# jmaronas/TGP.pytorch

Measured on AMD Instinct MI355X. Metric: ELBO-steps/sec (N x M kernel + chol + flow), Power M=100 S=32, higher is better.
Workload: dtype f64; 1 GPU; tgp_power_tanh3x2; rows_per_gpu=8611, D=4, M=100, S=32, flow=tanh3x2, parallelism=row-shard x1, launch=hipgraph, 40 / 10 steps per graph launch, replicas=1

## Files before the change

tgp/pytorch_amd/csrc/tgp_dev.hpp:

```cpp
#pragma once
#include <utility>
#include <hip/hip_runtime.h>
#include <stdint.h>
#include "../../../include/tgp_hip.h"

typedef double d4 __attribute__((ext_vector_type(4)));
#define TGP_MFMA(a, b, c) __builtin_amdgcn_mfma_f64_16x16x4f64((a), (b), (c), 0, 0, 0)

#define TGP_ROWS_PER_BLOCK 64
#define TGP_TILE_LD 66
#define TGP_MAX_MT 8
#ifndef TGP_RSPLIT
#define TGP_RSPLIT 4
#endif
#define TGP_LOG_2PI_REF 1.8378770942368803

#ifdef TGP_STAMPS
#define TGP_STAMP(wsp, plan, i)                                                                       \
  do {                                                                                                \
    if (blockIdx.x == 0 && threadIdx.x == 0)                                                          \
      (wsp)[(plan).hdr + tgp::H_STAMP + (i)] = (double)__builtin_amdgcn_s_memrealtime();              \
  } while (0)
#else
#define TGP_STAMP(wsp, plan, i) \
// ... 21 lines not shown
  size_t nD;
  size_t Gp;
  size_t redp;
  size_t PP;
  int PPW;
  size_t dbg;
  size_t slabs;
  size_t total;
};

enum { H_S2 = 0, H_KL = 1, H_ETA = 2, H_EINV = 3, H_SIG_OS = 4, H_STEP = 5, H_STAMP = 8, H_PSTAMP = 32, H_OUT = 60, H_N = 64 };
enum { C_ELL = 0, C_ETAB = 1, C_SVB = 2, C_PAD = 3, C_THETA = 4 };

inline size_t rup(size_t x, size_t a) { return (x + a - 1) / a * a; }

inline int rows4_waves(int N, int MT) {
  if ((N + 15) / 16 + MT <= 255) return 4;
  if ((N + 31) / 32 + MT <= 255) return 8;
  return 0;
}
inline int rows_rw(int N) { return (N > 4000 && (N + 39) / 40 <= 256) ? 10 : 16; }
inline int plan_alloc_blocks(int N) {
  int nb = (N + TGP_ROWS_PER_BLOCK - 1) / TGP_ROWS_PER_BLOCK;
  const int nw = rows4_waves(N, 1);
  if (nw > 0 && (N + 4 * nw - 1) / (4 * nw) > nb) nb = (N + 4 * nw - 1) / (4 * nw);
  const int rw = rows_rw(N);
  if ((N + 4 * rw - 1) / (4 * rw) > nb) nb = (N + 4 * rw - 1) / (4 * rw);
  return nb < 1 ? 1 : nb;
}

inline int make_plan(Plan& p, int N, int D, int M, int S, int nblk, int P, int RP, int lik, int nw4 = 0, int rw = 16) {
  if (D < 1 || D > 16) return -2;
  if (M < 1 || M > 16 * TGP_MAX_MT) return TGP_E_UNSUPPORTED;
  p.N = N; p.D = D; p.M = M; p.S = S; p.nblk = nblk; p.P = P; p.RP = RP; p.lik = lik; p.nslots = 0; p.zs_lds = 0;
  p.MT = (M + 15) / 16; p.MP = p.MT * 16;
  p.DP = D <= 4 ? 4 : (D <= 8 ? 8 : 16);
  p.CT = (2 * p.DP + 1 + 15) / 16; p.CT16 = p.CT * 16;
  p.ntri = p.MT * (p.MT + 1) / 2;
  p.nw4 = nw4;
  p.rw = rw;
  p.rpb = nw4 > 0 ? 4 * nw4 : 4 * rw;
  p.nblocks = (N + p.rpb - 1) / p.rpb;
  if (p.nblocks < 1) p.nblocks = 1;
  p.slab_G = 0;
  p.slab_T = p.slab_G + (size_t)p.ntri * 256;
  p.slab_S = p.slab_T + (size_t)p.MP * p.CT16;
  p.slab_C = p.slab_S + p.MP;
  p.slab_len = rup(p.slab_C + C_THETA + P, 16);
  size_t o = 0;
  const size_t mm = (size_t)p.MP * p.MP;
  p.hdr = o; o += H_N;
  p.ils = o; o += 16;
  p.ls = o; o += 16;
  p.Zs = o; o += (size_t)p.MP * p.DP;
  p.mpad = o; o += p.MP;
  p.w = o; o += p.MP;
  p.tp = o; o += rup(P + 1, 16);
  p.tg = o; o += rup(P + 1, 16);
  p.Kmm = o; o += mm; p.L = o; o += mm; p.J = o; o += mm; p.LT = o; o += mm;
  p.Lq = o; o += mm; p.LqT = o; o += mm; p.S_ = o; o += mm; p.HpT = o; o += mm; p.Q = o; o += mm;
  p.nD = o; o += (size_t)p.MT * 256;
  p.Gp = o; o += mm;
  p.redp = o; o += p.slab_len;
  p.PPW = p.DP + 2;
  p.PP = o; o += (size_t)2 * p.MT * p.MP * p.PPW;
  p.dbg = o; o += 256;
  p.slabs = o; o += (size_t)p.nblocks * p.slab_len;
  p.total = o;
  return 0;
}


__device__ __forceinline__ double exp_fast(double x) {
  x = fmin(fmax(x, -745.0), 709.0);
  const double k = rint(x * 1.4426950408889634074);
  double r = fma(-k, 6.93147180369123816490e-01, x);
  r = fma(-k, 1.90821492927058770002e-10, r);
  const double r2 = r * r, r4 = r2 * r2, r8 = r4 * r4;
  const double p01 = 1.0 + r;
  const double p23 = fma(r, 1.0 / 6.0, 0.5);
  const double p45 = fma(r, 1.0 / 120.0, 1.0 / 24.0);
  const double p67 = fma(r, 1.0 / 5040.0, 1.0 / 720.0);
  const double p89 = fma(r, 1.0 / 362880.0, 1.0 / 40320.0);
  const double pab = fma(r, 1.0 / 39916800.0, 1.0 / 3628800.0);
  const double pcd = fma(r, 1.0 / 6227020800.0, 1.0 / 479001600.0);
  const double q0 = fma(p23, r2, p01), q1 = fma(p67, r2, p45), q2 = fma(pab, r2, p89);
  const double s0 = fma(q1, r4, q0), s1 = fma(pcd, r4, q2);
  return ldexp(fma(s1, r8, s0), (int)k);
}

#define TGP_SQRT3 1.7320508075688772
__device__ __forceinline__ double cov_value(int kernel, double s2, double d2) {
  if (kernel == TGP_KERNEL_SCALE_MATERN32) {
    const double ar = TGP_SQRT3 * sqrt(fmax(d2, 1e-30));
    return s2 * (1.0 + ar) * exp_fast(-ar);
  }
  return s2 * exp_fast(-0.5 * d2);
}
__device__ __forceinline__ double cov_gweight(int kernel, double s2, double d2) {
  if (kernel == TGP_KERNEL_SCALE_MATERN32) return 3.0 * s2 * exp_fast(-TGP_SQRT3 * sqrt(fmax(d2, 1e-30)));
  return s2 * exp_fast(-0.5 * d2);
}

__device__ __forceinline__ double rsqrt_nr_fwd(double d) {
  double y = __builtin_amdgcn_rsq(d);
  const double h = 0.5 * d;
  y = y * fma(-h * y, y, 1.5);
  y = y * fma(-h * y, y, 1.5);
  return y;
}

__device__ __forceinline__ double log_fast(double x) {
  double m = __builtin_amdgcn_frexp_mant(x);
  int e = __builtin_amdgcn_frexp_exp(x);
  const bool lo = m < 0.70710678118654752440;
  m = lo ? m + m : m;
  e = lo ? e - 1 : e;
  const double den = m + 1.0;
  double y = __builtin_amdgcn_rcp(den);
  y = fma(fma(-den, y, 1.0), y, y);
  y = fma(fma(-den, y, 1.0), y, y);
  const double num = m - 1.0;
  double s_ = num * y;
  s_ = fma(fma(-den, s_, num), y, s_);
  const double z = s_ * s_, z2 = z * z, z4 = z2 * z2;
  const double p01 = fma(z, 2.0 / 5.0, 2.0 / 3.0);
  const double p23 = fma(z, 2.0 / 9.0, 2.0 / 7.0);
  const double p45 = fma(z, 2.0 / 13.0, 2.0 / 11.0);
  const double p67 = fma(z, 2.0 / 17.0, 2.0 / 15.0);
  const double p8 = 2.0 / 19.0;
  const double q0 = fma(p23, z2, p01), q1 = fma(p67, z2, p45);
  const double P = fma(fma(p8, z4, q1), z4, q0);
  const double lm = fma(s_ * z, P, s_ + s_);
  const double ed = (double)e;
  return fma(ed, 6.93147180369123816490e-01, fma(ed, 1.90821492927058770002e-10, lm));
}

__device__ __forceinline__ double rcp_fast(double x) {
  double y = __builtin_amdgcn_rcp(x);
  y = fma(fma(-x, y, 1.0), y, y);
  y = fma(fma(-x, y, 1.0), y, y);
  return y;
}

__device__ __forceinline__ double softplus_d(double x) {
  if (x > 20.0) return x;
  const double e = exp_fast(x), u = 1.0 + e;
  if (u == 1.0) return e;
  return log_fast(u) * (e * rcp_fast(u - 1.0));
}
__device__ __forceinline__ double sigmoid_d(double x) { return 1.0 / (1.0 + exp_fast(-x)); }

#define TGP_EACH(u, N) _Pragma("unroll") for (int u = 0; u < (N); ++u)
template <int N>
__device__ __forceinline__ void exp_fast_n(double (&x)[N]) {
  double k[N], r[N], r2[N], r4[N], r8[N], p01[N], p23[N], p45[N], p67[N], p89[N], pab[N], pcd[N];
  TGP_EACH(u, N) x[u] = fmin(fmax(x[u], -745.0), 709.0);
  TGP_EACH(u, N) k[u] = rint(x[u] * 1.4426950408889634074);
  TGP_EACH(u, N) r[u] = fma(-k[u], 6.93147180369123816490e-01, x[u]);
  TGP_EACH(u, N) r[u] = fma(-k[u], 1.90821492927058770002e-10, r[u]);
  TGP_EACH(u, N) r2[u] = r[u] * r[u];
  TGP_EACH(u, N) p01[u] = 1.0 + r[u];
  TGP_EACH(u, N) p23[u] = fma(r[u], 1.0 / 6.0, 0.5);
  TGP_EACH(u, N) p45[u] = fma(r[u], 1.0 / 120.0, 1.0 / 24.0);
  TGP_EACH(u, N) p67[u] = fma(r[u], 1.0 / 5040.0, 1.0 / 720.0);
  TGP_EACH(u, N) p89[u] = fma(r[u], 1.0 / 362880.0, 1.0 / 40320.0);
  TGP_EACH(u, N) pab[u] = fma(r[u], 1.0 / 39916800.0, 1.0 / 3628800.0);
  TGP_EACH(u, N) pcd[u] = fma(r[u], 1.0 / 6227020800.0, 1.0 / 479001600.0);
  TGP_EACH(u, N) r4[u] = r2[u] * r2[u];
  TGP_EACH(u, N) p01[u] = fma(p23[u], r2[u], p01[u]);
  TGP_EACH(u, N) p45[u] = fma(p67[u], r2[u], p45[u]);
  TGP_EACH(u, N) p89[u] = fma(pab[u], r2[u], p89[u]);
  TGP_EACH(u, N) r8[u] = r4[u] * r4[u];
  TGP_EACH(u, N) p01[u] = fma(p45[u], r4[u], p01[u]);
  TGP_EACH(u, N) p89[u] = fma(pcd[u], r4[u], p89[u]);
  TGP_EACH(u, N) x[u] = ldexp(fma(p89[u], r8[u], p01[u]), (int)k[u]);
}
template <int N>
__device__ __forceinline__ void rcp_fast_n(double (&x)[N]) {
  double y[N];
  TGP_EACH(u, N) y[u] = __builtin_amdgcn_rcp(x[u]);
  TGP_EACH(u, N) y[u] = fma(fma(-x[u], y[u], 1.0), y[u], y[u]);
  TGP_EACH(u, N) x[u] = fma(fma(-x[u], y[u], 1.0), y[u], y[u]);
}
template <int N>
__device__ __forceinline__ void rsqrt_nr_fwd_n(const double (&d)[N], double (&y)[N]) {
  TGP_EACH(u, N) y[u] = __builtin_amdgcn_rsq(d[u]);
  TGP_EACH(u, N) y[u] = y[u] * fma(-(0.5 * d[u]) * y[u], y[u], 1.5);
  TGP_EACH(u, N) y[u] = y[u] * fma(-(0.5 * d[u]) * y[u], y[u], 1.5);
}
template <int N>
__device__ __forceinline__ void log_fast_n(double (&x)[N]) {
  double m[N], den[N], y[N], num[N], s_[N], z[N], z2[N], z4[N], p01[N], p23[N], p45[N], p67[N], ed[N];
  TGP_EACH(u, N) {
    m[u] = __builtin_amdgcn_frexp_mant(x[u]);
    int e = __builtin_amdgcn_frexp_exp(x[u]);
    const bool lo = m[u] < 0.70710678118654752440;
    m[u] = lo ? m[u] + m[u] : m[u];
    e = lo ? e - 1 : e;
    ed[u] = (double)e;
  }
  TGP_EACH(u, N) den[u] = m[u] + 1.0;
  TGP_EACH(u, N) num[u] = m[u] - 1.0;
  TGP_EACH(u, N) y[u] = __builtin_amdgcn_rcp(den[u]);
  TGP_EACH(u, N) y[u] = fma(fma(-den[u], y[u], 1.0), y[u], y[u]);
  TGP_EACH(u, N) y[u] = fma(fma(-den[u], y[u], 1.0), y[u], y[u]);
  TGP_EACH(u, N) s_[u] = num[u] * y[u];
  TGP_EACH(u, N) s_[u] = fma(fma(-den[u], s_[u], num[u]), y[u], s_[u]);
  TGP_EACH(u, N) z[u] = s_[u] * s_[u];
  TGP_EACH(u, N) z2[u] = z[u] * z[u];
  TGP_EACH(u, N) p01[u] = fma(z[u], 2.0 / 5.0, 2.0 / 3.0);
  TGP_EACH(u, N) p23[u] = fma(z[u], 2.0 / 9.0, 2.0 / 7.0);
  TGP_EACH(u, N) p45[u] = fma(z[u], 2.0 / 13.0, 2.0 / 11.0);
  TGP_EACH(u, N) p67[u] = fma(z[u], 2.0 / 17.0, 2.0 / 15.0);
  TGP_EACH(u, N) z4[u] = z2[u] * z2[u];
  TGP_EACH(u, N) p01[u] = fma(p23[u], z2[u], p01[u]);
  TGP_EACH(u, N) p45[u] = fma(p67[u], z2[u], p45[u]);
  TGP_EACH(u, N) p45[u] = fma(2.0 / 19.0, z4[u], p45[u]);
  TGP_EACH(u, N) p01[u] = fma(p45[u], z4[u], p01[u]);
  TGP_EACH(u, N) p01[u] = fma(s_[u] * z[u], p01[u], s_[u] + s_[u]);
  TGP_EACH(u, N) x[u] = fma(ed[u], 6.93147180369123816490e-01, fma(ed[u], 1.90821492927058770002e-10, p01[u]));
}

__device__ __forceinline__ double xor_sum16(double x) {
  const unsigned lo = __double2loint(x), hi = __double2hiint(x);
  const auto a = __builtin_amdgcn_permlane16_swap(lo, lo, false, false);
  const auto b = __builtin_amdgcn_permlane16_swap(hi, hi, false, false);
  return __hiloint2double(b[0], a[0]) + __hiloint2double(b[1], a[1]);
}
__device__ __forceinline__ double xor_sum32(double x) {
  const unsigned lo = __double2loint(x), hi = __double2hiint(x);
  const auto a = __builtin_amdgcn_permlane32_swap(lo, lo, false, false);
  const auto b = __builtin_amdgcn_permlane32_swap(hi, hi, false, false);
  return __hiloint2double(b[0], a[0]) + __hiloint2double(b[1], a[1]);
}
__device__ __forceinline__ double quad_sum(double x) { return xor_sum32(xor_sum16(x)); }
template <int R>
__device__ __forceinline__ double ror_sum(double x) {
  const int lo = __double2loint(x), hi = __double2hiint(x);
  const int l2 = __builtin_amdgcn_update_dpp(0, lo, 0x120 + R, 0xf, 0xf, false);
  const int h2 = __builtin_amdgcn_update_dpp(0, hi, 0x120 + R, 0xf, 0xf, false);
  return x + __hiloint2double(h2, l2);
}
__device__ __forceinline__ double wave_sum(double x) {
  x = xor_sum16(xor_sum32(x));
  return ror_sum<1>(ror_sum<2>(ror_sum<4>(ror_sum<8>(x))));
}

template <int K>
__device__ __forceinline__ double bcast_row_k(double x) {
  return __builtin_amdgcn_update_dpp(0.0, x, 0x150 + K, 0xf, 0xf, true);
}
template <class F, int... Is>
__device__ __forceinline__ void static_for_impl(F&& f, std::integer_sequence<int, Is...>) {
  (f(std::integral_constant<int, Is>{}), ...);
}
template <int N, class F>
__device__ __forceinline__ void static_for(F&& f) {
  static_for_impl(static_cast<F&&>(f), std::make_integer_sequence<int, N>{});
}

__device__ __forceinline__ double rsqrt_nr(double d) {
  double y = __builtin_amdgcn_rsq(d);
  const double h = 0.5 * d;
  y = y * fma(-h * y, y, 1.5);
  y = y * fma(-h * y, y, 1.5);
  return y;
}

__device__ __forceinline__ int potrf_trtri16(double (&a)[16], double (&x)[16], int lane) {
  int bad = 0;
  static_for<16>([&](auto kc) {
    constexpr int k = decltype(kc)::value;
    const double d = bcast_row_k<k>(a[k]);
    if (!(d > 0.0) && bad == 0) bad = k + 1;
    const double rinv = rsqrt_nr(d);
    double s0 = 0.0, s1 = 0.0;
    static_for<16>([&](auto mc) {
      constexpr int m = decltype(mc)::value;
      if constexpr (m < k) {
        if constexpr ((m & 1) == 0) s0 = fma(bcast_row_k<k>(a[m]), x[m], s0);
        else s1 = fma(bcast_row_k<k>(a[m]), x[m], s1);
      }
    });
    x[k] = (lane == k) ? rinv : (lane < k ? -(s0 + s1) * rinv : 0.0);
    a[k] = (lane == k) ? d * rinv : a[k] * rinv;
    static_for<16>([&](auto jc) {
      constexpr int j = decltype(jc)::value;
      if constexpr (j > k) {
        a[j] = fma(-a[k], bcast_row_k<j>(a[k]), a[j]);
        asm volatile("" : "+v"(a[j]));
      }
    });
  });
  return bad;
}

template <bool PANEL, bool TRTRI = false, bool RDIAG = false>
__device__ __forceinline__ int potrf_panel16(double (&dg)[16], double (&a)[16], double* x = nullptr, int lane = 0,
                                             double* rd = nullptr) {
  int bad = 0;
  static_for<16>([&](auto kc) {
    constexpr int k = decltype(kc)::value;
    const double d = bcast_row_k<k>(dg[k]);
    if (!(d > 0.0) && bad == 0) bad = k + 1;
    const double rinv = rsqrt_nr(d);
// ... 818 lines not shown
```

tgp/pytorch_amd/csrc/tgp_mm.hip:

```cpp
#include "tgp_dev.hpp"
#include "tgp_prep.hpp"
#include "tgp_launch.hpp"

namespace tgp {

#define PREP_THREADS 512
#ifndef TGP_W4_WINDOWS
#define TGP_W4_WINDOWS 2
#endif

__global__ __launch_bounds__(PREP_THREADS) void k_prep_a(Plan p, tgp_model md, FlowProg fp, double* __restrict__ ws,
                                                         int32_t* __restrict__ status) {
  extern __shared__ __attribute__((aligned(16))) unsigned char smem_raw[];
  double* sm = reinterpret_cast<double*>(smem_raw);
  const int tid = threadIdx.x, lane = tid & 63;
  const int wave = __builtin_amdgcn_readfirstlane(tid >> 6);
  const int r = lane & 15, q = lane >> 4;
  const int M = p.M, D = p.D, MP = p.MP, DP = p.DP, MT = p.MT;

  int32_t* sy = status + 4;
  const int nb_total = 3 + MT * MT;
  if ((int)blockIdx.x < MT * MT) {
    prep_tile_role<PREP_THREADS, true>(p, md, ws, (int)blockIdx.x, sy);
    sync_leave(sy, nb_total);
    return;
  }

  if ((int)blockIdx.x == MT * MT) {
    prep_xform_role<PREP_THREADS, false>(p, md, fp, ws);
    sync_leave(sy, nb_total);
    return;
  }

  const int cb = (int)blockIdx.x - (MT * MT + 1);
  constexpr int NW = PREP_THREADS / 64;
  const int LD = MP + 1;
  double* A = sm;
  double* zs = sm + (size_t)MP * LD;
  __shared__ int s_info, s_nan, s_next, s_sync;
  __shared__ double s_ils[16];
  if (tid == 0) { s_info = 0; s_nan = 0; s_next = 0; s_sync = 0; }
  int tbase = 0;
  if (tid < 16) s_ils[tid] = tid < D ? 1.0 / softplus_d(md.raw_ls[tid]) : 0.0;
  const double s2 = softplus_d(md.raw_os[0]);
  const bool zl = p.zs_lds != 0;
  if (zl) {
    for (int i = tid; i < MP * DP; i += PREP_THREADS) {
      const int mrow = i / DP, d = i % DP;
      zs[i] = (mrow < M && d < D) ? md.Z[(size_t)mrow * D + d] * (1.0 / softplus_d(md.raw_ls[d])) : 0.0;
    }
  }
  __syncthreads();
  bool has_nan = false;
  double jit = md.jitter;
  auto kmm_elem = [&](int rr, int cc) {
    double k;
    if (rr < M) {
      double d2 = 0.0;
      if (zl) {
        for (int d = 0; d < DP; d += 4) {
          const double2 a0 = *reinterpret_cast<const double2*>(zs + rr * DP + d), a1 = *reinterpret_cast<const double2*>(zs + rr * DP + d + 2);
          const double2 b0 = *reinterpret_cast<const double2*>(zs + cc * DP + d), b1 = *reinterpret_cast<const double2*>(zs + cc * DP + d + 2);
          const double t0 = a0.x - b0.x, t1 = a0.y - b0.y, t2 = a1.x - b1.x, t3 = a1.y - b1.y;
          d2 += t0 * t0; d2 += t1 * t1; d2 += t2 * t2; d2 += t3 * t3;
        }
      } else {
        for (int d = 0; d < D; ++d) {
          const double tt = (md.Z[(size_t)rr * D + d] - md.Z[(size_t)cc * D + d]) * s_ils[d];
          d2 += tt * tt;
        }
      }
      k = s2 * exp_fast(-0.5 * d2);
      has_nan |= (k != k);
      if (rr == cc) k += jit;
    } else {
      k = (rr == cc) ? 1.0 : 0.0;
    }
    return k;
  };
  auto ll_sum = [&](int i0, int j0, int kbeg, int kend) {
    d4 acc = {0, 0, 0, 0};
    return tile_mm_f([&](int k) { return A[(i0 + r) * LD + k + q]; }, [&](int k) { return A[(j0 + r) * LD + k + q]; }, kbeg,
                     kend, acc);
  };
  auto write_L = [&](int ti, int tj) {
#pragma unroll
    for (int u = 0; u < 4; ++u) {
      const int rr = 16 * ti + q + 4 * u, cc = 16 * tj + r;
      ws[p.L + (size_t)rr * MP + cc] = (ti != tj || cc <= rr) ? A[rr * LD + cc] : 0.0;
      const int rt = 16 * tj + q + 4 * u, ct = 16 * ti + r;
      ws[p.LT + (size_t)rt * MP + ct] = (ti != tj || rt <= ct) ? A[ct * LD + rt] : 0.0;
    }
  };
  auto inv_diag = [&](int jt) {
    const int li = lane & 15;
    double dgv[16], xv[16];
#pragma unroll
    for (int c = 0; c < 16; ++c) dgv[c] = A[(16 * jt + li) * LD + 16 * jt + c];
    trtri16(dgv, xv, li);
#pragma unroll
    for (int u = 0; u < 4; ++u) {
      const double xv4 = q == 0 ? xv[4 * u] : (q == 1 ? xv[4 * u + 1] : (q == 2 ? xv[4 * u + 2] : xv[4 * u + 3]));
      ws[p.nD + jt * 256 + (4 * u + q) * 16 + li] = -xv4;
    }
  };
  auto sub16 = [&](int i, int c, int k0) {
    double a4[4], b4[4];
#pragma unroll
    for (int s4 = 0; s4 < 4; ++s4) { a4[s4] = A[(16 * i + r) * LD + k0 + 4 * s4 + q]; b4[s4] = A[(16 * c + r) * LD + k0 + 4 * s4 + q]; }
    double cur[4];
#pragma unroll
    for (int rr = 0; rr < 4; ++rr) cur[rr] = A[(16 * i + q + 4 * rr) * LD + 16 * c + r];
    d4 acc = {0, 0, 0, 0};
#pragma unroll
    for (int s4 = 0; s4 < 4; ++s4) acc = TGP_MFMA(a4[s4], b4[s4], acc);
#pragma unroll
    for (int rr = 0; rr < 4; ++rr) A[(16 * i + q + 4 * rr) * LD + 16 * c + r] = cur[rr] - acc[rr];
  };
  const double* __restrict__ Kg = ws + p.Kmm;
  bool tiles_seen = false;
  auto fill_tile = [&](int i, int c, int ncol) {
    double kv[4];
    if (c >= 2) {
      if (!tiles_seen) {
        const int v = sync_wait(sy + SY_TILES, [&](int x) { return (x & 0xffff) >= MT * MT; });
        if (v == (int)0x80000000 && lane == 0) s_sync = 1;
        tiles_seen = true;
      }
#pragma unroll
      for (int u = 0; u < 4; ++u) kv[u] = ld_agent(Kg + (size_t)(16 * i + q + 4 * u) * MP + 16 * c + r);
#pragma unroll
      for (int u = 0; u < 4; ++u) {
        const int rr = 16 * i + q + 4 * u, cc = 16 * c + r;
        has_nan |= (kv[u] != kv[u]);
        if (rr == cc) kv[u] = rr < M ? kv[u] + jit : 1.0;
      }
    } else if (zl) {
      const int cc = 16 * c + r;
      double e[4];
      TGP_EACH(u, 4) {
        const int rr = 16 * i + q + 4 * u;
        double d2 = 0.0;
        for (int d = 0; d < DP; d += 4) {
          const double2 a0 = *reinterpret_cast<const double2*>(zs + rr * DP + d), a1 = *reinterpret_cast<const double2*>(zs + rr * DP + d + 2);
          const double2 b0 = *reinterpret_cast<const double2*>(zs + cc * DP + d), b1 = *reinterpret_cast<const double2*>(zs + cc * DP + d + 2);
          const double t0 = a0.x - b0.x, t1 = a0.y - b0.y, t2 = a1.x - b1.x, t3 = a1.y - b1.y;
          d2 += t0 * t0; d2 += t1 * t1; d2 += t2 * t2; d2 += t3 * t3;
        }
        e[u] = -0.5 * d2;
      }
      exp_fast_n<4>(e);
      TGP_EACH(u, 4) {
        const int rr = 16 * i + q + 4 * u;
        double k = s2 * e[u];
        has_nan |= (rr < M) && (k != k);
        if (rr == cc) k += jit;
        kv[u] = rr < M ? k : (rr == cc ? 1.0 : 0.0);
      }
    } else {
#pragma unroll
      for (int u = 0; u < 4; ++u) kv[u] = kmm_elem(16 * i + q + 4 * u, 16 * c + r);
    }
    if (ncol > 0) {
      const d4 upd = ll_sum(16 * i, 16 * c, 0, 16 * ncol);
#pragma unroll
      for (int u = 0; u < 4; ++u) kv[u] -= upd[u];
    }
#pragma unroll
    for (int u = 0; u < 4; ++u) A[(16 * i + q + 4 * u) * LD + 16 * c + r] = kv[u];
  };
#define PREP_BARRIER() asm volatile("s_waitcnt lgkmcnt(0)\n\ts_barrier" ::: "memory")
#ifdef TGP_STAMPS
  double tph[10] = {0, 0, 0, 0, 0, 0, 0, 0, 0, 0};
  double tcnt[6] = {0, 0, 0, 0, 0, 0};
  unsigned long long tl_ = 0;
#define PSTAMP0() do { __builtin_amdgcn_sched_barrier(0); tl_ = __builtin_amdgcn_s_memtime(); __builtin_amdgcn_sched_barrier(0); } while (0)
#define PSTAMP(i) do { __builtin_amdgcn_sched_barrier(0); unsigned long long tn_ = __builtin_amdgcn_s_memtime(); __builtin_amdgcn_sched_barrier(0); tph[i] += (double)(tn_ - tl_); tl_ = tn_; } while (0)
#else
#define PSTAMP0() do { } while (0)
#define PSTAMP(i) do { } while (0)
#endif
  int attempt = 0;
  PSTAMP0();
  for (;; ++attempt) {
    if (wave < MT) fill_tile(wave, 0, 0);
    PREP_BARRIER();
    PSTAMP(0);
    for (int j = 0; j < MT; ++j) {
      const int j0 = 16 * j;
      const int npan = (MT - 1 - j) * 16;
      const int npw = npan > 64 ? 2 : (npan > 0 ? 1 : 0);
      double ltile[4] = {0.0, 0.0, 0.0, 0.0};
      bool did_diag = false;
      if (wave < npw || (npw == 0 && wave == 0)) {
        __builtin_amdgcn_s_setprio(3);
        const int li = lane & 15, l0 = wave * 64 + lane;
        const bool has = l0 < npan;
        const int prow = j0 + (npan > 0 ? 16 : 0) + (has ? l0 : 0);
        double dg[16], a[16];
#pragma unroll
        for (int c = 0; c < 16; ++c) dg[c] = A[(j0 + li) * LD + j0 + c];
        if (npan > 0) {
#pragma unroll
          for (int c = 0; c < 16; ++c) a[c] = A[prow * LD + j0 + c];
        }
#ifdef TGP_STAMPS
        asm volatile("s_waitcnt lgkmcnt(0)" ::: "memory");
#endif
        PSTAMP(1);
        int bad = 0;
        if (npan > 0) bad = potrf_panel16<true>(dg, a);
        else bad = potrf_panel16<false>(dg, a);
#ifdef TGP_STAMPS
        asm volatile("" ::"v"(dg[15]), "v"(a[15]));
#endif
        PSTAMP(2);
        if (has && npan > 0) {
#pragma unroll
          for (int c = 0; c < 16; ++c) A[prow * LD + j0 + c] = a[c];
        }
        if (wave == 0) {
#pragma unroll
          for (int u = 0; u < 4; ++u)
            ltile[u] = q == 0 ? dg[4 * u] : (q == 1 ? dg[4 * u + 1] : (q == 2 ? dg[4 * u + 2] : dg[4 * u + 3]));
          did_diag = true;
          if (lane == 0 && bad != 0 && s_info == 0) s_info = j0 + bad;
        }
#ifdef TGP_STAMPS
        asm volatile("s_waitcnt lgkmcnt(0)" ::: "memory");
#endif
        PSTAMP(3);
        __builtin_amdgcn_s_setprio(0);
#ifdef TGP_STAMPS
        if (wave != 0) { tph[j == 0 ? 7 : 8] += tph[1] + tph[2] + tph[3]; tph[1] = tph[2] = tph[3] = 0.0; }
#endif
      } else if (wave != 4 || j < TGP_W4_WINDOWS) {
        const int nt = (j >= 1 && ((j - 1) & 1) == cb) ? 1 : 0;
        const int nf = MT - 1 - j;
        const int nwl = (j + 1 - cb) / 2;
        const int ntask = nt + nf + nwl;
        for (;;) {
          int t = 0;
          if (lane == 0) t = atomicAdd(&s_next, 1);
          t = __builtin_amdgcn_readfirstlane(t) - tbase;
          if (t >= ntask) break;
          if (t < nt) { inv_diag(j - 1); continue; }
          t -= nt;
          if (t < nf) { fill_tile(j + 1 + t, j + 1, j); continue; }
          t -= nf;
          write_L(j - 1, 2 * t + cb);
        }
#ifdef TGP_STAMPS
        asm volatile("s_waitcnt lgkmcnt(0)" ::: "memory");
        if (j == 0) PSTAMP(7); else PSTAMP(8);
#endif
      }
      tbase += ((j >= 1 && ((j - 1) & 1) == cb) ? 1 : 0) + (MT - 1 - j) + (j + 1 - cb) / 2 +
               (NW - (j < TGP_W4_WINDOWS ? 0 : 1) - (npw > 0 ? npw : 1));
      PREP_BARRIER();
      PSTAMP(4);
      if (did_diag) {
#pragma unroll
        for (int u = 0; u < 4; ++u) A[(j0 + (lane & 15)) * LD + j0 + 4 * u + q] = ltile[u];
      }
      if (j + 1 < MT) {
        for (int i = j + 1 + wave; i < MT; i += NW) sub16(i, j + 1, j0);
#ifdef TGP_STAMPS
        asm volatile("s_waitcnt lgkmcnt(0)" ::: "memory");
#endif
        PSTAMP(5);
        PREP_BARRIER();
        PSTAMP(6);
      }
    }
    if (has_nan) s_nan = 1;
    __syncthreads();
    if (s_info == 0 || s_nan != 0 || !(md.jitter_ladder > 0.0) || attempt == 3) break;
    __syncthreads();
    if (tid == 0) s_info = 0;
    jit = md.jitter + md.jitter_ladder * (attempt == 0 ? 1.0 : (attempt == 1 ? 10.0 : 100.0));
    __syncthreads();
  }
  if (((MT - 1) & 1) == cb && wave == NW - 1) inv_diag(MT - 1);
  for (int t = wave; t < (MT + 1 - cb) / 2; t += NW) write_L(MT - 1, 2 * t + cb);
  PSTAMP(9);
#ifdef TGP_STAMPS
  if (lane == 0) {
    if (wave == 0)
      for (int i = 0; i < 10; ++i) ws[p.hdr + H_PSTAMP + i] = tph[i];
    if (wave == 3) for (int i = 1; i <= 5; ++i) { ws[p.hdr + H_PSTAMP + 26 + i] = tph[i]; ws[p.hdr + 20 + i] = tcnt[i]; }
    ws[p.hdr + H_PSTAMP + 10 + 2 * wave] = tph[7];
    ws[p.hdr + H_PSTAMP + 11 + 2 * wave] = tph[8];
  }
#endif
  if (tid == 0 && cb == 0) {
    status[0] = s_sync != 0 ? TGP_STATUS_SYNC_TIMEOUT : s_info;
    if (s_sync != 0) __hip_atomic_fetch_add(status + 3, 1, __ATOMIC_RELAXED, __HIP_MEMORY_SCOPE_AGENT);
    status[1] = s_nan;
    status[2] = s_info == 0 ? attempt : 0;
  }
  sync_leave(sy, nb_total);
#undef PREP_BARRIER
}

size_t prep_a_lds_bytes(const Plan& p) {
  return ((size_t)p.MP * (p.MP + 1) + (p.zs_lds ? (size_t)p.MP * p.DP : 0) + 16) * sizeof(double);
}

#define RED_ELEMS (256 / TGP_RSPLIT)
__global__ __launch_bounds__(256) void k_reduce(Plan p, double* __restrict__ ws) {
#ifdef TGP_STAMPS
  if (blockIdx.x == 0 && threadIdx.x == 0) ws[p.dbg + 200 + 16] = (double)__builtin_amdgcn_s_memrealtime();
#endif
  __shared__ double part_s[TGP_RSPLIT][RED_ELEMS];
  const int tid = threadIdx.x, sh = tid / RED_ELEMS, el = tid % RED_ELEMS;
  const size_t e = (size_t)blockIdx.x * RED_ELEMS + el;
  const bool in = e < p.slab_len;
  const int b0 = (int)((long long)p.nblocks * sh / TGP_RSPLIT), b1 = (int)((long long)p.nblocks * (sh + 1) / TGP_RSPLIT);
  const double* sl = ws + p.slabs + (in ? e : 0);
  constexpr int RB = 28;
  double s0 = 0.0, s1 = 0.0, s2 = 0.0, s3 = 0.0;
  for (int b = b0; b < b1; b += RB) {
    double t[RB];
#pragma unroll
    for (int u = 0; u < RB; ++u) {
      const int bu = b + u < b1 ? b + u : b1 - 1;
      t[u] = sl[(size_t)bu * p.slab_len];
    }
#pragma unroll
    for (int u = 0; u < RB; ++u) t[u] = b + u < b1 ? t[u] : 0.0;
#pragma unroll
    for (int u = 0; u < RB; u += 4) { s0 += t[u]; s1 += t[u + 1]; s2 += t[u + 2]; s3 += t[u + 3]; }
  }
  part_s[sh][el] = b1 > b0 ? (s0 + s1) + (s2 + s3) : 0.0;
  __syncthreads();
  if (sh != 0 || !in) return;
  double s = 0.0;
#pragma unroll
  for (int k = 0; k < TGP_RSPLIT; ++k) s += part_s[k][el];
  if (e < p.slab_T) {
    const int t = (int)(e >> 8), in_t = (int)(e & 255), row = in_t >> 4, col = in_t & 15;
    int ti = 0;
    while ((ti + 1) * (ti + 2) / 2 <= t) ++ti;
    const int tj = t - ti * (ti + 1) / 2;
    if (ti == tj && col > row) return;
    double* G = ws + p.Gp;
    st_wt(&G[(size_t)(ti * 16 + row) * p.MP + tj * 16 + col], s);
    st_wt(&G[(size_t)(tj * 16 + col) * p.MP + ti * 16 + row], s);
  } else {
    st_wt(&ws[p.redp + e], s);
  }
}

__device__ __forceinline__ double red_tail(const Plan& p, const double* __restrict__ ws, size_t e) { return ws[p.redp + e]; }

#define BWD_THREADS 512
#define TGP_PF2 32

__device__ __forceinline__ void adam_elem(const AdamDev& A, long i, double g, double pi, double mi, double vi, double bc1,
                                          double bc2s) {
  const double gi = A.sign * g;
  const double m1 = A.b1 * mi + (1.0 - A.b1) * gi;
  const double v1 = A.b2 * vi + (1.0 - A.b2) * gi * gi;
  A.m[i] = m1;
  A.v[i] = v1;
  A.p[i] = pi - (A.lr / bc1) * m1 / (sqrt(v1) / bc2s + A.eps);
}

enum { SB_PROG = 0, SB_LEFT = 1 };
#ifdef TGP_STAMPS
#define BW_STAMP(on, i) do { if ((on) && threadIdx.x == 0) ws[p.dbg + 200 + (i)] = (double)__builtin_amdgcn_s_memrealtime(); } while (0)
#else
#define BW_STAMP(on, i) do { } while (0)
#endif

__device__ __forceinline__ void bwd_leave(int32_t* sb) {
  __syncthreads();
  if (threadIdx.x == 0) sync_add(sb + SB_LEFT, 1);
}

__device__ __forceinline__ void report_sync_timeout(int32_t* __restrict__ status) {
  __hip_atomic_store(status, (int32_t)TGP_STATUS_SYNC_TIMEOUT, __ATOMIC_RELAXED, __HIP_MEMORY_SCOPE_AGENT);
  __hip_atomic_fetch_add(status + 3, 1, __ATOMIC_RELAXED, __HIP_MEMORY_SCOPE_AGENT);
}
template <class P>
__device__ __forceinline__ void bwd_wait(const int32_t* w, P pred, int32_t* __restrict__ status) {
  if (threadIdx.x < 64) {
    const int v = sync_wait(w, pred);
    if (v == (int)0x80000000 && threadIdx.x == 0) {
      report_sync_timeout(status);
      asm volatile("s_waitcnt vmcnt(0)" ::: "memory");
    }
  }
  __syncthreads();
}
__device__ __forceinline__ bool bwd_timed_out(const int32_t* __restrict__ status) {
  return __hip_atomic_load(status, __ATOMIC_RELAXED, __HIP_MEMORY_SCOPE_AGENT) == (int32_t)TGP_STATUS_SYNC_TIMEOUT;
}

typedef double bwd_d2 __attribute__((ext_vector_type(2)));
#define BWD_G_NIT ((8 * TGP_MAX_MT * 16 + BWD_THREADS - 1) / BWD_THREADS)
__device__ __forceinline__ void bwd_g_issue(const Plan& p, const double* __restrict__ ws, int c0,
                                            bwd_d2 (&gv)[BWD_G_NIT], double& sv0) {
  const int MP = p.MP, tid = threadIdx.x;
  const double* __restrict__ Gp = ws + p.Gp;
#pragma unroll
  for (int u = 0; u < BWD_G_NIT; ++u) {
    const int i = tid + u * BWD_THREADS;
    const int ic = i < MP * 8 ? i : 0;
    gv[u] = *reinterpret_cast<const bwd_d2*>(Gp + (size_t)(ic >> 3) * MP + c0 + 2 * (ic & 7));
  }
  sv0 = tid < 16 ? red_tail(p, ws, p.slab_S + c0 + tid) : 0.0;
}
__device__ __forceinline__ void bwd_g_commit(const Plan& p, double* Gs, double* LbL, double* svL,
                                             const bwd_d2 (&gv)[BWD_G_NIT], double sv0) {
  const int MP = p.MP, tid = threadIdx.x;
#pragma unroll
  for (int u = 0; u < BWD_G_NIT; ++u) {
    const int i = tid + u * BWD_THREADS;
    if (i < MP * 8) {
      reinterpret_cast<bwd_d2*>(Gs)[i] = gv[u];
      reinterpret_cast<bwd_d2*>(LbL)[i] = bwd_d2{0.0, 0.0};
    }
  }
  if (tid < 16) svL[tid] = sv0;
}

template <int PF, bool SWAP = false, class FB>
__device__ __forceinline__ d4 tile_mm_regA(const double (&a)[PF], FB fb, int n, d4 acc) {
#pragma unroll
  for (int s0 = 0; s0 < PF; s0 += 8) {
    if (s0 < n) {
      double o[8];
#pragma unroll
      for (int u = 0; u < 8; ++u) o[u] = s0 + u < n ? fb(s0 + u) : 0.0;
#pragma unroll
      for (int u = 0; u < 8; ++u)
        if (s0 + u < n) acc = SWAP ? TGP_MFMA(o[u], a[s0 + u], acc) : TGP_MFMA(a[s0 + u], o[u], acc);
    }
  }
  return acc;
}

__device__ __forceinline__ void bwd_lam_role(const Plan& p, const tgp_model& md, const tgp_grads& g, double* __restrict__ ws,
                                             const AdamDev& ad, double* sm, int c, const int32_t* __restrict__ status) {
  static_assert(TGP_MAX_MT <= BWD_THREADS / 64, "one tile per wave");
  const int MP = p.MP, MT = p.MT, M = p.M;
  double* Gs = sm;
  double* LbL = Gs + (size_t)MP * 16;
  double* svL = LbL + (size_t)MP * 16;
  const int tid = threadIdx.x, lane = tid & 63, wave = __builtin_amdgcn_readfirstlane(tid >> 6), r = lane & 15, q = lane >> 4;
  const int c0 = 16 * c;
  BW_STAMP(c == 0, 4);
  bwd_d2 gv[BWD_G_NIT];
  double sv0;
  bwd_g_issue(p, ws, c0, gv, sv0);
  constexpr int PF = TGP_PF2;
  const double* __restrict__ Lq = ws + p.Lq;
  const int j = wave, j0 = 16 * j;
// ... 422 lines not shown
  __syncthreads();
  for (int i = tid; i < N2 * D; i += 256) {
    const int c = i / D, d = i - c * D;
    zT[d * N2 + c] = X2[i] * ils[d];
  }
  for (int i = tid; i < nr * D; i += 256) {
    const int r = i / D, d = i - r * D;
    xT[d * COVF_ROWS + r] = X1[n0 * D + i] * ils[d];
  }
  __syncthreads();
  const double s2 = ils[16];
  const int npairs = nr * (N2 / 2);
  const int sr = 512 / N2, sc = 512 - sr * N2;
  int e = 2 * tid, r = e / N2, c = e - r * N2;
  double* __restrict__ Ko = K + n0 * (long)N2;
  for (int p = tid; p < npairs; p += 512) {
    int r1 = r + sr, c1 = c + sc;
    if (c1 >= N2) { c1 -= N2; ++r1; }
    const bool has1 = p + 256 < npairs;
    const int rb = has1 ? r1 : r, cb = has1 ? c1 : c;
    double ev[4] = {0.0, 0.0, 0.0, 0.0};
    for (int d = 0; d < D; ++d) {
      const double xa = xT[d * COVF_ROWS + r], xb = xT[d * COVF_ROWS + rb];
      const double2 za = *reinterpret_cast<const double2*>(zT + d * N2 + c);
      const double2 zb = *reinterpret_cast<const double2*>(zT + d * N2 + cb);
      const double t0 = xa - za.x, t1 = xa - za.y, t2 = xb - zb.x, t3 = xb - zb.y;
      ev[0] += t0 * t0; ev[1] += t1 * t1; ev[2] += t2 * t2; ev[3] += t3 * t3;
    }
    if (kernel == TGP_KERNEL_SCALE_RBF) {
      TGP_EACH(u, 4) ev[u] *= -0.5;
      exp_fast_n<4>(ev);
      TGP_EACH(u, 4) ev[u] *= s2;
    } else {
      TGP_EACH(u, 4) ev[u] = cov_value(kernel, s2, ev[u]);
    }
    if (self) {
      if (n0 + r == c) ev[0] += jitter;
      if (n0 + r == c + 1) ev[1] += jitter;
      if (n0 + rb == cb) ev[2] += jitter;
      if (n0 + rb == cb + 1) ev[3] += jitter;
    }
    *reinterpret_cast<double2*>(Ko + e) = make_double2(ev[0], ev[1]);
    if (has1) *reinterpret_cast<double2*>(Ko + e + 512) = make_double2(ev[2], ev[3]);
    r = r1 + sr; c = c1 + sc;
    if (c >= N2) { c -= N2; ++r; }
    e += 1024;
  }
}

__global__ __launch_bounds__(256) void k_kl(const double* __restrict__ m, const double* __restrict__ Lam, int M,
                                             double* __restrict__ out, double* __restrict__ g_m,
                                             double* __restrict__ g_Lam) {
  __shared__ double wsum[4];
  const int tid = threadIdx.x;
  double part = 0.0;
  for (int it = tid; it < M * M; it += 256) {
    const int r = it / M, c = it % M;
    double gl = 0.0;
    if (c <= r) {
      const double x = Lam[it];
      part += x * x;
      gl = x;
      if (c == r) { part -= log(x * x); gl = x - 1.0 / x; }
    }
    if (g_Lam) g_Lam[it] = gl;
  }
  for (int i = tid; i < M; i += 256) {
    part += m[i] * m[i];
    if (g_m) g_m[i] = m[i];
  }
  part = wave_sum(part);
  if ((tid & 63) == 0) wsum[tid >> 6] = part;
  __syncthreads();
  if (tid == 0) out[0] = 0.5 * (wsum[0] + wsum[1] + wsum[2] + wsum[3] - (double)M);
}

__global__ void k_unpad(const double* __restrict__ src, int MP, int M, double* __restrict__ dst) {
  const int i = blockIdx.x * blockDim.x + threadIdx.x;
  if (i >= M * M) return;
  dst[i] = src[(size_t)(i / M) * MP + i % M];
}

__global__ __launch_bounds__(PREP_THREADS) void k_chol_only(const double* __restrict__ Ain, int M, int MP,
                                                            double* __restrict__ Lout, double* __restrict__ Jout,
                                                            int32_t* __restrict__ status) {
  extern __shared__ __attribute__((aligned(16))) unsigned char smem_raw[];
  double* A = reinterpret_cast<double*>(smem_raw);
  const int LD = MP + 1;
  double* dinv = A + (size_t)MP * LD;
  __shared__ int s_info, s_nan;
  const int tid = threadIdx.x;
  if (tid == 0) { s_info = 0; s_nan = 0; }
  __syncthreads();
  bool has_nan = false;
  for (int i = tid; i < M * M; i += PREP_THREADS) {
    const double x = Ain[i];
    has_nan |= (x != x);
    A[(i / M) * LD + i % M] = x;
  }
  if (has_nan) s_nan = 1;
  for (int j = 0; j < M; ++j) {
    __syncthreads();
    const double d = A[j * LD + j];
    if (!(d > 0.0)) {
      if (tid == 0 && s_info == 0) s_info = j + 1;
    }
    const double dj = sqrt(d), inv = 1.0 / dj;
    __syncthreads();
    for (int i = j + tid; i < M; i += PREP_THREADS) A[i * LD + j] = (i == j) ? dj : A[i * LD + j] * inv;
    __syncthreads();
    const int rem = M - j - 1;
    for (int e = tid; e < rem * rem; e += PREP_THREADS) {
      const int i = j + 1 + e / rem, k = j + 1 + e % rem;
      if (k <= i) A[i * LD + k] -= A[i * LD + j] * A[k * LD + j];
    }
  }
  __syncthreads();
  if (tid < M) dinv[tid] = 1.0 / A[tid * LD + tid];
  __syncthreads();
  if (Jout != nullptr && tid < M) {
    const int c = tid;
    for (int i = c + 1; i < M; ++i) {
      double s = A[i * LD + c] * dinv[c];
      for (int k = c + 1; k < i; ++k) s += A[i * LD + k] * A[c * LD + k];
      A[c * LD + i] = -s * dinv[i];
    }
  }
  __syncthreads();
  for (int i = tid; i < M * M; i += PREP_THREADS) {
    const int r = i / M, c = i % M;
    double l = 0.0, jv = 0.0;
    if (c < r) { l = A[r * LD + c]; jv = A[c * LD + r]; }
    else if (c == r) { l = A[r * LD + r]; jv = dinv[r]; }
    Lout[i] = l;
    if (Jout != nullptr) Jout[i] = jv;
  }
  if (tid == 0) { status[0] = s_info; status[1] = s_nan; }
}

#define LAUNCH_CHECK()                                   \
  do {                                                   \
    hipError_t e_ = hipGetLastError();                   \
    if (e_ != hipSuccess) return set_error(e_, __FILE__, __LINE__); \
  } while (0)

int launch_prepare(const Plan& p_in, const tgp_model& md, const FlowProg& fp, double* ws, int32_t* status,
                   hipStream_t st) {
  Plan p = p_in;
  p.zs_lds = 1;
  if (prep_a_lds_bytes(p) > 160 * 1024 - 1024) p.zs_lds = 0;
  const size_t lds = prep_a_lds_bytes(p);
  static size_t lds_cur = 48 * 1024;
  if (int rc = ensure_lds(reinterpret_cast<const void*>(k_prep_a), lds, &lds_cur)) return rc;
  hipLaunchKernelGGL(k_prep_a, dim3(3 + p.MT * p.MT), dim3(PREP_THREADS), lds, st, p, md, fp, ws, status);
  LAUNCH_CHECK();
  return 0;
}

int launch_backward_mm(const Plan& p, const tgp_model& md, const tgp_grads& g, double* out, double* ws, int32_t* status,
                       hipStream_t st, const AdamDev* adam) {
  const AdamDev ad = adam != nullptr ? *adam : AdamDev();
  hipLaunchKernelGGL(k_reduce, dim3((unsigned)((p.slab_len + RED_ELEMS - 1) / RED_ELEMS)), dim3(256), 0, st, p, ws);
  LAUNCH_CHECK();
  const size_t lds_col = (size_t)(2 * p.MP * 16 + 16), lds_row = (size_t)p.MT * 256 + 16 * p.DP + (size_t)p.MP * 16,
               lds_fin = (size_t)p.M * (p.D + 1) + (adam != nullptr && ad.n - ad.lam_n <= BWD_MIRROR_MAX ? (size_t)(ad.n - ad.lam_n) : 0) + p.M;
  const size_t lds = sizeof(double) * (lds_col > lds_row ? (lds_col > lds_fin ? lds_col : lds_fin) : (lds_row > lds_fin ? lds_row : lds_fin));
  hipLaunchKernelGGL(k_bwd, dim3(4 * p.MT + 1), dim3(BWD_THREADS), lds, st, p, md, g, out, ws, ad, status);
  LAUNCH_CHECK();
  return 0;
}

static int launch_cov_tile(int kernel, const double* X1, int N1, const double* X2, int N2, int D, const double* raw_ls,
                           const double* raw_os, double jitter, int self, double* K, hipStream_t st) {
  if (D < 1 || D > 16) return TGP_E_UNSUPPORTED;
  if (N1 < 1 || N2 < 1) return 0;
  if ((N2 & 1) == 0 && N2 >= 2 && (long)N2 * D <= 4096 && N2 <= 512 && (reinterpret_cast<uintptr_t>(K) & 15) == 0) {
    const unsigned gx = (unsigned)((N1 + COVF_ROWS - 1) / COVF_ROWS);
    const size_t lds = ((size_t)D * N2 + (size_t)D * COVF_ROWS) * sizeof(double);
    static size_t lds_cur = 48 * 1024;
    if (int rc = ensure_lds(reinterpret_cast<const void*>(k_cov_flat), lds, &lds_cur)) return rc;
    hipLaunchKernelGGL(k_cov_flat, dim3(gx), dim3(256), lds, st, kernel, X1, N1, X2, N2, D, raw_ls, raw_os, jitter, self, K);
    LAUNCH_CHECK();
    return 0;
  }
  const unsigned gx = (unsigned)((N1 + COV_ROWS - 1) / COV_ROWS), gy = (unsigned)((N2 + COV_COLS - 1) / COV_COLS);
  if (gy > 65535u) return TGP_E_UNSUPPORTED;
  hipLaunchKernelGGL(k_cov_tile, dim3(gx, gy), dim3(256), 0, st, kernel, X1, N1, X2, N2, D, raw_ls, raw_os, jitter, self, K);
  LAUNCH_CHECK();
  return 0;
}

int launch_kmm(const double* Z, const double* raw_ls, const double* raw_os, int M, int D, double jitter, double* K,
               hipStream_t st) {
  return launch_cov_tile(TGP_KERNEL_SCALE_RBF, Z, M, Z, M, D, raw_ls, raw_os, jitter, 1, K, st);
}

int launch_knm(const double* X, const double* Z, const double* raw_ls, const double* raw_os, int N, int M, int D,
               double* K, hipStream_t st) {
  return launch_cov_tile(TGP_KERNEL_SCALE_RBF, X, N, Z, M, D, raw_ls, raw_os, 0.0, 0, K, st);
}

int launch_kernel_matrix(int kernel, const double* X1, int N1, const double* X2, int N2, int D, const double* raw_ls,
                         const double* raw_os, double jitter, double* K, hipStream_t st) {
  if (X2 == nullptr) return launch_cov_tile(kernel, X1, N1, X1, N1, D, raw_ls, raw_os, jitter, 1, K, st);
  return launch_cov_tile(kernel, X1, N1, X2, N2, D, raw_ls, raw_os, 0.0, 0, K, st);
}

int launch_kl(const double* m, const double* Lam, int M, double* out, double* g_m, double* g_Lam, hipStream_t st) {
  hipLaunchKernelGGL(k_kl, dim3(1), dim3(256), 0, st, m, Lam, M, out, g_m, g_Lam);
  LAUNCH_CHECK();
  return 0;
}

int launch_cholesky(const double* A, int M, double* L, double* Linv, int32_t* status, hipStream_t st) {
  const int MP = (M + 15) / 16 * 16;
  const size_t lds = ((size_t)MP * (MP + 1) + MP) * sizeof(double);
  static size_t lds_cur = 48 * 1024;
  if (int rc = ensure_lds(reinterpret_cast<const void*>(k_chol_only), lds, &lds_cur)) return rc;
  hipLaunchKernelGGL(k_chol_only, dim3(1), dim3(PREP_THREADS), lds, st, A, M, MP, L, Linv, status);
  LAUNCH_CHECK();
  return 0;
}

}
```

Measured before the change: 10660 ELBO-steps/s.

## Split Cholesky prep across four redundant blocks and vectorise LDS row loads

The redundant Cholesky blocks in k_prep_a go from 2 to 4 (PREP_NCB). Each block now writes out a quarter of the L/LT tiles and diagonal inverses instead of half, which shortens the write-out tail. The LDS row stride becomes MP+2 so rows are 16-byte aligned, and the 16-element row loads and stores are done as double2 accesses to cut LDS instruction count. The cost is two more blocks each repeating the whole factorisation, slightly more LDS, and changed bank mapping from the new stride.

```diff
diff --git a/tgp/pytorch_amd/csrc/tgp_dev.hpp b/tgp/pytorch_amd/csrc/tgp_dev.hpp
--- a/tgp/pytorch_amd/csrc/tgp_dev.hpp
+++ b/tgp/pytorch_amd/csrc/tgp_dev.hpp
@@ -197,6 +197,18 @@
 __device__ __forceinline__ double sigmoid_d(double x) { return 1.0 / (1.0 + exp_fast(-x)); }
 
 #define TGP_EACH(u, N) _Pragma("unroll") for (int u = 0; u < (N); ++u)
+__device__ __forceinline__ void lds_row16(const double* __restrict__ src, double (&v)[16]) {
+  const double2* s2 = reinterpret_cast<const double2*>(src);
+  TGP_EACH(c, 8) {
+    const double2 t = s2[c];
+    v[2 * c] = t.x;
+    v[2 * c + 1] = t.y;
+  }
+}
+__device__ __forceinline__ void lds_store_row16(double* __restrict__ dst, const double (&v)[16]) {
+  double2* d2 = reinterpret_cast<double2*>(dst);
+  TGP_EACH(c, 8) d2[c] = make_double2(v[2 * c], v[2 * c + 1]);
+}
 template <int N>
 __device__ __forceinline__ void exp_fast_n(double (&x)[N]) {
   double k[N], r[N], r2[N], r4[N], r8[N], p01[N], p23[N], p45[N], p67[N], p89[N], pab[N], pcd[N];
diff --git a/tgp/pytorch_amd/csrc/tgp_mm.hip b/tgp/pytorch_amd/csrc/tgp_mm.hip
--- a/tgp/pytorch_amd/csrc/tgp_mm.hip
+++ b/tgp/pytorch_amd/csrc/tgp_mm.hip
@@ -5,6 +5,7 @@
 namespace tgp {
 
 #define PREP_THREADS 512
+#define PREP_NCB 4
 #ifndef TGP_W4_WINDOWS
 #define TGP_W4_WINDOWS 2
 #endif
@@ -19,7 +20,7 @@
   const int M = p.M, D = p.D, MP = p.MP, DP = p.DP, MT = p.MT;
 
   int32_t* sy = status + 4;
-  const int nb_total = 3 + MT * MT;
+  const int nb_total = 1 + PREP_NCB + MT * MT;
   if ((int)blockIdx.x < MT * MT) {
     prep_tile_role<PREP_THREADS, true>(p, md, ws, (int)blockIdx.x, sy);
     sync_leave(sy, nb_total);
@@ -34,7 +35,7 @@
 
   const int cb = (int)blockIdx.x - (MT * MT + 1);
   constexpr int NW = PREP_THREADS / 64;
-  const int LD = MP + 1;
+  const int LD = MP + 2;
   double* A = sm;
   double* zs = sm + (size_t)MP * LD;
   __shared__ int s_info, s_nan, s_next, s_sync;
@@ -95,8 +96,7 @@
   auto inv_diag = [&](int jt) {
     const int li = lane & 15;
     double dgv[16], xv[16];
-#pragma unroll
-    for (int c = 0; c < 16; ++c) dgv[c] = A[(16 * jt + li) * LD + 16 * jt + c];
+    lds_row16(A + (16 * jt + li) * LD + 16 * jt, dgv);
     trtri16(dgv, xv, li);
 #pragma unroll
     for (int u = 0; u < 4; ++u) {
@@ -198,12 +198,8 @@
         const bool has = l0 < npan;
         const int prow = j0 + (npan > 0 ? 16 : 0) + (has ? l0 : 0);
         double dg[16], a[16];
-#pragma unroll
-        for (int c = 0; c < 16; ++c) dg[c] = A[(j0 + li) * LD + j0 + c];
-        if (npan > 0) {
-#pragma unroll
-          for (int c = 0; c < 16; ++c) a[c] = A[prow * LD + j0 + c];
-        }
+        lds_row16(A + (j0 + li) * LD + j0, dg);
+        if (npan > 0) lds_row16(A + prow * LD + j0, a);
 #ifdef TGP_STAMPS
         asm volatile("s_waitcnt lgkmcnt(0)" ::: "memory");
 #endif
@@ -215,10 +211,7 @@
         asm volatile("" ::"v"(dg[15]), "v"(a[15]));
 #endif
         PSTAMP(2);
-        if (has && npan > 0) {
-#pragma unroll
-          for (int c = 0; c < 16; ++c) A[prow * LD + j0 + c] = a[c];
-        }
+        if (has && npan > 0) lds_store_row16(A + prow * LD + j0, a);
         if (wave == 0) {
 #pragma unroll
           for (int u = 0; u < 4; ++u)
@@ -235,9 +228,9 @@
         if (wave != 0) { tph[j == 0 ? 7 : 8] += tph[1] + tph[2] + tph[3]; tph[1] = tph[2] = tph[3] = 0.0; }
 #endif
       } else if (wave != 4 || j < TGP_W4_WINDOWS) {
-        const int nt = (j >= 1 && ((j - 1) & 1) == cb) ? 1 : 0;
+        const int nt = (j >= 1 && (j - 1) % PREP_NCB == cb) ? 1 : 0;
         const int nf = MT - 1 - j;
-        const int nwl = (j + 1 - cb) / 2;
+        const int nwl = (j + PREP_NCB - 1 - cb) / PREP_NCB;
         const int ntask = nt + nf + nwl;
         for (;;) {
           int t = 0;
@@ -248,14 +241,14 @@
           t -= nt;
           if (t < nf) { fill_tile(j + 1 + t, j + 1, j); continue; }
           t -= nf;
-          write_L(j - 1, 2 * t + cb);
+          write_L(j - 1, PREP_NCB * t + cb);
         }
 #ifdef TGP_STAMPS
         asm volatile("s_waitcnt lgkmcnt(0)" ::: "memory");
         if (j == 0) PSTAMP(7); else PSTAMP(8);
 #endif
       }
-      tbase += ((j >= 1 && ((j - 1) & 1) == cb) ? 1 : 0) + (MT - 1 - j) + (j + 1 - cb) / 2 +
+      tbase += ((j >= 1 && (j - 1) % PREP_NCB == cb) ? 1 : 0) + (MT - 1 - j) + (j + PREP_NCB - 1 - cb) / PREP_NCB +
                (NW - (j < TGP_W4_WINDOWS ? 0 : 1) - (npw > 0 ? npw : 1));
       PREP_BARRIER();
       PSTAMP(4);
@@ -281,11 +274,11 @@
     jit = md.jitter + md.jitter_ladder * (attempt == 0 ? 1.0 : (attempt == 1 ? 10.0 : 100.0));
     __syncthreads();
   }
-  if (((MT - 1) & 1) == cb && wave == NW - 1) inv_diag(MT - 1);
-  for (int t = wave; t < (MT + 1 - cb) / 2; t += NW) write_L(MT - 1, 2 * t + cb);
+  if ((MT - 1) % PREP_NCB == cb && wave == NW - 1) inv_diag(MT - 1);
+  for (int t = wave; t < (MT + PREP_NCB - 1 - cb) / PREP_NCB; t += NW) write_L(MT - 1, PREP_NCB * t + cb);
   PSTAMP(9);
 #ifdef TGP_STAMPS
-  if (lane == 0) {
+  if (lane == 0 && cb == 0) {
     if (wave == 0)
       for (int i = 0; i < 10; ++i) ws[p.hdr + H_PSTAMP + i] = tph[i];
     if (wave == 3) for (int i = 1; i <= 5; ++i) { ws[p.hdr + H_PSTAMP + 26 + i] = tph[i]; ws[p.hdr + 20 + i] = tcnt[i]; }
@@ -304,7 +297,7 @@
 }
 
 size_t prep_a_lds_bytes(const Plan& p) {
-  return ((size_t)p.MP * (p.MP + 1) + (p.zs_lds ? (size_t)p.MP * p.DP : 0) + 16) * sizeof(double);
+  return ((size_t)p.MP * (p.MP + 2) + (p.zs_lds ? (size_t)p.MP * p.DP : 0) + 16) * sizeof(double);
 }
 
 #define RED_ELEMS (256 / TGP_RSPLIT)
@@ -1033,7 +1026,7 @@
   const size_t lds = prep_a_lds_bytes(p);
   static size_t lds_cur = 48 * 1024;
   if (int rc = ensure_lds(reinterpret_cast<const void*>(k_prep_a), lds, &lds_cur)) return rc;
-  hipLaunchKernelGGL(k_prep_a, dim3(3 + p.MT * p.MT), dim3(PREP_THREADS), lds, st, p, md, fp, ws, status);
+  hipLaunchKernelGGL(k_prep_a, dim3(1 + PREP_NCB + p.MT * p.MT), dim3(PREP_THREADS), lds, st, p, md, fp, ws, status);
   LAUNCH_CHECK();
   return 0;
 }
```

Result: no change. 10730 ELBO-steps/s, median of 6 (+0.7%).
